# SeoYeonnLee/Video-Chapter-Generation

Measured on AMD Instinct MI355X. Metric: clip-windows/sec (16f×224²+128tok) train-step at 1/2/4/8 MI355X; % HBM roofline, higher is better.
Workload: dtype bf16; 1 GPU; TwoStream train step: TSM-ResNet-50 + BERT-base + ChapterHead(mlp), B=64 windows/GPU of 16x224^2 frames + 128 tokens, fused clip+AdamW; global_batch=64, seq_len=128, frames=16, resolution=224, text_fill=n_valid ~ U[L/2, L], parallelism=dp1

## Files before the change

### video-chapter-generation_amd/csrc/igemm_wide.hip

```cpp
#include "fastload.h"

namespace vcg {

namespace {

__device__ __forceinline__ int w_xcd_slot(int b, int n) {
  const int q = n >> 3, r = n & 7, x = b & 7;
  return (x < r ? x * (q + 1) : r * (q + 1) + (x - r) * q) + (b >> 3);
}

}

enum { WE_STORE = 0, WE_GELU = 1, WE_GELU_BWD = 2, WE_RES = 3, WE_RES32 = 4 };

namespace {

__device__ const float4 g_wide_zero4 = {0.f, 0.f, 0.f, 0.f};

template <int MT, int NT, int WE>
__device__ __forceinline__ void wide_epilogue(f32x4 (&acc)[MT][NT], const GemmParams& p, int m0, int n0) {
  bf16_t* C = reinterpret_cast<bf16_t*>(p.C);
  const bf16_t* R = reinterpret_cast<const bf16_t*>(p.residual);
  float rv[MT][NT][4];
  if constexpr (WE == WE_GELU_BWD || WE == WE_RES || WE == WE_RES32) {
#pragma unroll
    for (int j = 0; j < NT; ++j)
#pragma unroll
      for (int i = 0; i < MT; ++i) {
        const int m = min(m0 + i * 16, p.M - 1), n = min(n0 + j * 16, p.N - 4);
        if constexpr (WE == WE_RES32)
          load4<float>(reinterpret_cast<const float*>(p.residual) + (long long)m * p.ldr + n, rv[i][j]);
        else
          load4<bf16_t>(R + (long long)m * p.ldr + n, rv[i][j]);
      }
  }
#pragma unroll
  for (int j = 0; j < NT; ++j) {
    const int n = n0 + j * 16;
    const float4* bp = p.bias ? reinterpret_cast<const float4*>(p.bias + min(n, p.N - 4)) : &g_wide_zero4;
    const float4 b4 = *bp;
    const float bv[4] = {b4.x, b4.y, b4.z, b4.w};
#pragma unroll
    for (int i = 0; i < MT; ++i) {
      const int m = m0 + i * 16;
      float v[4];
#pragma unroll
      for (int r = 0; r < 4; ++r) {
        float t = acc[i][j][r] + bv[r];
        if constexpr (WE == WE_GELU) {
          v[r] = p.fast_act ? gelu_erf_fast(t) : gelu_erf(t);
          acc[i][j][r] = t;
        } else if constexpr (WE == WE_GELU_BWD) {
          t = bf2f(f2bf(t));
          v[r] = t * (p.fast_act ? gelu_erf_grad_fast(rv[i][j][r]) : gelu_erf_grad(rv[i][j][r]));
        } else if constexpr (WE == WE_RES || WE == WE_RES32) {
          v[r] = t + rv[i][j][r];
        } else {
          v[r] = t;
        }
      }
      if (m < p.M && n < p.N) {
        if constexpr (WE == WE_RES32)
          store4<float>(reinterpret_cast<float*>(p.C) + (long long)m * p.ldc + n, v);
        else
          store4<bf16_t>(C + (long long)m * p.ldc + n, v);
        if constexpr (WE == WE_GELU) {
          if (p.aux) {
            const float a4[4] = {acc[i][j][0], acc[i][j][1], acc[i][j][2], acc[i][j][3]};
            store4<bf16_t>(reinterpret_cast<bf16_t*>(p.aux) + (long long)m * p.ldc + n, a4);
          }
        }
      }
    }
  }
}

}

#ifdef VCG_WIDE_STAMPS
__device__ unsigned long long g_wide_stamps[2 * 16 * 2 * 4];
#define W_STAMP(s, ph, k)                                                                                      \
  do {                                                                                                         \
    if (blockIdx.x == 0 && (tid == 0 || tid == 256) && (s) >= 8 && (s) < 24)                                  \
      g_wide_stamps[((((tid >> 8) * 16 + (s) - 8) * 2 + (ph)) * 4) + (k)] = __builtin_amdgcn_s_memtime();      \
  } while (0)
#else
#define W_STAMP(s, ph, k) do {} while (0)
#endif
#ifndef VCG_WIDE_ABL
#define VCG_WIDE_ABL 0
#endif

template <int P>
__device__ __forceinline__ void wide_wait(int ahead) {
  if (ahead >= 2) __builtin_amdgcn_s_waitcnt(waitcnt_vm(2 * P));
  else if (ahead == 1) __builtin_amdgcn_s_waitcnt(waitcnt_vm(P));
  else __builtin_amdgcn_s_waitcnt(waitcnt_vm(0));
}

template <int BM, int BN, int NW = 8>
struct WideLoader {
  static constexpr int PA = BM / (8 * NW), PB = BN / (8 * NW), P = PA + PB, AE = BM * FBK;
  __amdgpu_buffer_rsrc_t ra, rb;
  uint32_t oa, ob;
  int off[P];
  int kc[P];
  __device__ __forceinline__ void init(const GemmParams& p) {
    oa = (uint32_t)min(p.a.bytes, (long long)0xFFFFFF00LL);
    ob = (uint32_t)min(p.b.bytes, (long long)0xFFFFFF00LL);
    ra = __builtin_amdgcn_make_buffer_rsrc(const_cast<void*>(p.a.ptr), 0, oa, 0x00020000);
    rb = __builtin_amdgcn_make_buffer_rsrc(const_cast<void*>(p.b.ptr), 0, ob, 0x00020000);
  }
  __device__ __forceinline__ void tile(const GemmParams& p, int m0, int n0, int wave, int lane) {
#pragma unroll
    for (int q = 0; q < P; ++q) {
      const bool isa = q < PA;
      const int r = (wave * (isa ? PA : PB) + (isa ? q : q - PA)) * 8 + (lane >> 3);
      kc[q] = 8 * fswz(r, lane & 7);
      const int gr = (isa ? m0 : n0) + r;
      off[q] = gr < (isa ? p.M : p.N) ? (int)((long long)gr * (isa ? p.a.ld : p.b.ld)) + kc[q] : -1;
    }
  }
  template <int Q>
  __device__ __forceinline__ void piece(int k0, int K, bf16_t* stage, int wave) const {
    constexpr bool isa = Q < PA;
    const uint32_t bad = isa ? oa : ob;
    const uint32_t voff = (off[Q] >= 0 && k0 + kc[Q] < K) ? (uint32_t)(off[Q] + k0) * 2u : bad;
    bf16_t* slice = stage + (isa ? 0 : AE) + (wave * (isa ? PA : PB) + (isa ? Q : Q - PA)) * 512;
    __builtin_amdgcn_raw_ptr_buffer_load_lds(isa ? ra : rb, (lds_void_t*)slice, 16, voff, 0, 0, 0);
  }
  template <int Q = 0>
  __device__ __forceinline__ void all(int k0, int K, bf16_t* stage, int wave) const {
    if constexpr (Q < P) {
      piece<Q>(k0, K, stage, wave);
      all<Q + 1>(k0, K, stage, wave);
    }
  }
};

template <int BM, int BN, int WE, int ST = 3>
__global__ __launch_bounds__(512) void gemm_wide_kernel(GemmParams p) {
  constexpr int MT = BM / 32, NT = BN / 64;
  constexpr int AE = BM * FBK, BE = BN * FBK, SE = AE + BE;
  constexpr int PIECES = BM / 64 + BN / 64;
  constexpr int PF = ST - 1;
  static_assert(ST * SE * 2 <= 160 * 1024, "LDS");
  __shared__ __attribute__((aligned(1024))) bf16_t smem[ST * SE];
  const int tid = threadIdx.x, lane = tid & 63;
  const int wave = __builtin_amdgcn_readfirstlane(tid >> 6);
  const int grp = wave >> 2, wc = wave & 3;
  const int ntn = (p.N + BN - 1) / BN, ntm = (p.M + BM - 1) / BM, ntiles = ntn * ntm;
  const int G = gridDim.x;
  const int slot = w_xcd_slot(blockIdx.x, G);
  const int mine = slot < ntiles ? (ntiles - 1 - slot) / G + 1 : 0;
  const int nk = (p.K + FBK - 1) / FBK;
  const int steps = mine * nk;
  if (steps == 0) return;

  WideLoader<BM, BN> ld;
  ld.init(p);
  int ikt = 0, itile = 0;
  bf16_t* istage = smem;
  auto next_tile = [&]() {
    if (ikt == 0) {
      const int L = slot + itile * G, mt = L / ntn, nt = L - mt * ntn;
      ld.tile(p, mt * BM, nt * BN, wave, lane);
    }
  };
  auto advance = [&]() {
    if (++ikt == nk) {
      ikt = 0;
      ++itile;
    }
  };

  f32x4 acc[MT][NT];
#pragma unroll
  for (int i = 0; i < MT; ++i)
#pragma unroll
    for (int j = 0; j < NT; ++j) acc[i][j] = f32x4{0.f, 0.f, 0.f, 0.f};

#pragma unroll
  for (int t = 0; t < PF; ++t)
    if (t < steps) {
      next_tile();
      ld.all(ikt * FBK, p.K, smem + t * SE, wave);
      advance();
    }
  wide_wait<PIECES>(min(PF, steps) - 1);
  __builtin_amdgcn_s_barrier();
  if (grp == 1) __builtin_amdgcn_s_barrier();

  int cur = 0, kt = 0, tile = 0;
  s16x8 af[MT][2], bq[NT][2];
  for (int s = 0; s < steps; ++s) {
    const bf16_t* Ac = smem + cur * SE;
    const bf16_t* Bc = Ac + AE;
    const bool pre = s + PF < steps;
    if (pre) {
      next_tile();
      istage = smem + (cur == 0 ? ST - 1 : cur - 1) * SE;
    }
    const int ik0 = ikt * FBK;
    W_STAMP(s, 0, 0);
    if (VCG_WIDE_ABL != 3 || s == 0) {
#pragma unroll
      for (int s2 = 0; s2 < 2; ++s2) {
#pragma unroll
        for (int j = 0; j < NT; ++j) bq[j][s2] = fast_frag(Bc, wc * (BN / 4) + j * 16, lane, s2);
#pragma unroll
        for (int i = 0; i < MT; ++i) af[i][s2] = fast_frag(Ac, grp * (BM / 2) + i * 16, lane, s2);
      }
    }
    if (pre && VCG_WIDE_ABL != 1) ld.all(ik0, p.K, istage, wave);
    W_STAMP(s, 0, 1);
    __builtin_amdgcn_s_waitcnt(0xC07F);
    W_STAMP(s, 0, 2);
    if (grp == 1 && s + 1 < steps && VCG_WIDE_ABL != 1)
      wide_wait<PIECES>(min(s + PF, steps - 1) - (s + 1));
    W_STAMP(s, 0, 3);
    __builtin_amdgcn_s_barrier();
    W_STAMP(s, 1, 0);
    __builtin_amdgcn_sched_barrier(0);
    __builtin_amdgcn_s_setprio(1);
    if (VCG_WIDE_ABL != 2) {
#pragma unroll
      for (int s2 = 0; s2 < 2; ++s2)
#pragma unroll
        for (int i = 0; i < MT; ++i)
#pragma unroll
          for (int j = 0; j < NT; ++j)
            acc[i][j] = __builtin_amdgcn_mfma_f32_16x16x32_bf16(bq[j][s2], af[i][s2], acc[i][j], 0, 0, 0);
    }
    __builtin_amdgcn_s_setprio(0);
    if (pre) advance();
    W_STAMP(s, 1, 1);
    if (grp == 0 && s + 1 < steps && VCG_WIDE_ABL != 1) wide_wait<PIECES>(min(s + PF, steps - 1) - (s + 1));
    W_STAMP(s, 1, 2);
    __builtin_amdgcn_sched_barrier(0);
    if (++kt == nk) {
      const int L = slot + tile * G, mt = L / ntn, nt = L - mt * ntn;
      wide_epilogue<MT, NT, WE>(acc, p, mt * BM + grp * (BM / 2) + (lane & 15), nt * BN + wc * (BN / 4) + 4 * (lane >> 4));
#pragma unroll
      for (int i = 0; i < MT; ++i)
#pragma unroll
        for (int j = 0; j < NT; ++j) acc[i][j] = f32x4{0.f, 0.f, 0.f, 0.f};
      kt = 0;
      ++tile;
    }
    W_STAMP(s, 1, 3);
    __builtin_amdgcn_s_barrier();
    cur = cur == ST - 1 ? 0 : cur + 1;
  }
  if (grp == 0) __builtin_amdgcn_s_barrier();
}

namespace {

int wide_cus() {
  static int n = 0;
  if (n == 0) {
    int dev = 0, c = 0;
    if (hipGetDevice(&dev) == hipSuccess && hipDeviceGetAttribute(&c, hipDeviceAttributeMultiprocessorCount, dev) ==
                                                hipSuccess && c > 0)
      n = c;
    else
      n = 256;
  }
  return n;
}

int wide_bn_for(const GemmParams& p) {
  if (const char* e = getenv("VCG_WIDE_BN")) {
    const int v = atoi(e);
    if (v == 128 || v == 192 || v == 256) return v;
  }
  if (p.N >= 3072 && p.N % 256 == 0) return 256;
  return p.N % 192 == 0 ? 192 : 128;
}

template <int BN, int WE>
void launch_wide(const GemmParams& p, hipStream_t s) {
  constexpr int BM = 128;
  const long long tiles = (long long)((p.M + BM - 1) / BM) * ((p.N + BN - 1) / BN);
  const int grid = (int)(tiles < wide_cus() ? tiles : wide_cus());
  hipLaunchKernelGGL((gemm_wide_kernel<BM, BN, WE>), dim3(grid), dim3(512), 0, s, p);
}

template <int BN>
void launch_wide_we(const GemmParams& p, int we, hipStream_t s) {
  switch (we) {
    case WE_GELU: launch_wide<BN, WE_GELU>(p, s); break;
    case WE_GELU_BWD: launch_wide<BN, WE_GELU_BWD>(p, s); break;
    case WE_RES: launch_wide<BN, WE_RES>(p, s); break;
    case WE_RES32: launch_wide<BN, WE_RES32>(p, s); break;
    default: launch_wide<BN, WE_STORE>(p, s); break;
  }
}

}

int wide_gemm_class(const GemmParams& p) {
  if (p.alpha != 1.f || p.batch_inner > 0 || p.M <= 0 || p.N <= 0 || p.K <= 0) return -1;
  if (p.N % 8 != 0 || p.K % 8 != 0 || (p.ldc & 7) != 0 || (p.a.ld & 7) != 0 || (p.b.ld & 7) != 0) return -1;
  if ((((uintptr_t)p.C | (uintptr_t)p.a.ptr | (uintptr_t)p.b.ptr) & 15) != 0) return -1;
  if (p.a.bytes >= 0xFFFFFF00LL || p.b.bytes >= 0xFFFFFF00LL) return -1;
  if (p.bias && ((uintptr_t)p.bias & 15) != 0) return -1;
  if (p.aux && (p.act != ACT_GELU || ((uintptr_t)p.aux & 15) != 0)) return -1;
  if (p.residual) {
    if (p.residual == p.C || (p.ldr & 3) != 0 || ((uintptr_t)p.residual & 7) != 0) return -1;
    if (p.act == ACT_GELU_BWD) return WE_GELU_BWD;
    return p.act == ACT_NONE && !p.res_round ? WE_RES : -1;
  }
  if (p.act == ACT_GELU) return WE_GELU;
  return p.act == ACT_NONE ? WE_STORE : -1;
}

int wide_gemm_class_f32(const GemmParams& p) {
  if (!p.residual || p.aux || p.act != ACT_NONE || p.res_round || p.alpha != 1.f || p.batch_inner > 0) return -1;
  if (p.N % 8 != 0 || p.K % 8 != 0 || (p.ldc & 3) != 0 || (p.ldr & 3) != 0 || (p.a.ld & 7) != 0 || (p.b.ld & 7) != 0)
    return -1;
  if ((((uintptr_t)p.C | (uintptr_t)p.residual | (uintptr_t)p.a.ptr | (uintptr_t)p.b.ptr) & 15) != 0) return -1;
  if (p.a.bytes >= 0xFFFFFF00LL || p.b.bytes >= 0xFFFFFF00LL) return -1;
  if (p.bias && ((uintptr_t)p.bias & 15) != 0) return -1;
  return WE_RES32;
}

int run_gemm_wide(GemmParams& p, int we, hipStream_t s) {
  const int tk = timing_begin(s);
  switch (wide_bn_for(p)) {
    case 128: launch_wide_we<128>(p, we, s); break;
    case 256: launch_wide_we<256>(p, we, s); break;
    default: launch_wide_we<192>(p, we, s); break;
  }
  const double es = we == WE_RES32 ? 4.0 : 2.0;
  double bytes = 2.0 * ((double)p.M * p.K + (double)p.N * p.K) + es * p.M * (double)p.N;
  if (p.residual) bytes += es * p.M * (double)p.N;
  if (p.aux) bytes += 2.0 * p.M * (double)p.N;
  timing_end(tk, s, TIMING_WIDE_GEMM, 2.0 * p.M * p.N * (double)p.K, bytes);
  if (census_on()) { char t_[96]; snprintf(t_, sizeof(t_), "gemm_wide 128x%d we%d", wide_bn_for(p), we); census_add(t_, p.M, p.N, p.K); }
  VCG_LAUNCH_CHECK();
  return VCG_OK;
}

}

VCG_API int vcg_wide_stamps(unsigned long long* out, int n) {
#ifdef VCG_WIDE_STAMPS
  n = n < 256 ? n : 256;
  return hipMemcpyFromSymbol(out, HIP_SYMBOL(vcg::g_wide_stamps), (size_t)n * 8, 0, hipMemcpyDeviceToHost) == hipSuccess
             ? 0 : 2;
#else
  (void)out;
  (void)n;
  return 1;
#endif
}
```

Measured before the change: 913.0 clip-windows/sec.

## Restructure wide GEMM main loop to overlap fragment loads with MFMA halves

Reworks the persistent wide GEMM loop so each k-step splits into two MFMA halves. The second-half LDS fragments are read while the first half computes, and the next stage's first-half fragments are read after the barrier. Global prefetch is now issued after compute into the just-consumed stage, one barrier per step replaces the staggered group barriers, and bias/residual loads for the epilogue are issued early on the last k-step with vmcnt accounting. This is meant to hide LDS and epilogue load latency, but it relies on hand-counted waitcnts that are fixed to 3 stages.

```diff
diff --git a/video-chapter-generation_amd/csrc/igemm_wide.hip b/video-chapter-generation_amd/csrc/igemm_wide.hip
--- a/video-chapter-generation_amd/csrc/igemm_wide.hip
+++ b/video-chapter-generation_amd/csrc/igemm_wide.hip
@@ -1,3 +1,5 @@
+#include <type_traits>
+
 #include "fastload.h"
 
 namespace vcg {
@@ -15,30 +17,74 @@
 
 namespace {
 
-__device__ const float4 g_wide_zero4 = {0.f, 0.f, 0.f, 0.f};
-
-template <int MT, int NT, int WE>
-__device__ __forceinline__ void wide_epilogue(f32x4 (&acc)[MT][NT], const GemmParams& p, int m0, int n0) {
+
+template <int WE> struct WideRes { using T = uint2; };
+template <> struct WideRes<WE_RES32> { using T = float4; };
+constexpr bool wide_has_res(int we) { return we == WE_GELU_BWD || we == WE_RES || we == WE_RES32; }
+
+template <int MT, int NT, int WE>
+struct WideEpiOps {
+  float4 bias[NT];
+  typename WideRes<WE>::T res[MT][NT];
+};
+template <int MT, int NT, int WE>
+constexpr bool wide_res_early() {
+  return wide_has_res(WE) && MT * NT * (int)sizeof(typename WideRes<WE>::T) / 4 <= 48;
+}
+template <int MT, int NT, int WE>
+constexpr int wide_epi_loads() { return NT + (wide_res_early<MT, NT, WE>() ? MT * NT : 0); }
+
+template <int MT, int NT, int WE>
+__device__ __forceinline__ void wide_res_load(WideEpiOps<MT, NT, WE>& e, const GemmParams& p, int m0, int n0) {
+  using T = typename WideRes<WE>::T;
+  const char* R = reinterpret_cast<const char*>(p.residual);
+#pragma unroll
+  for (int j = 0; j < NT; ++j)
+#pragma unroll
+    for (int i = 0; i < MT; ++i) {
+      const int m = min(m0 + i * 16, p.M - 1), n = min(n0 + j * 16, p.N - 4);
+      e.res[i][j] = *reinterpret_cast<const T*>(R + ((long long)m * p.ldr + n) * (long long)(sizeof(T) / 4));
+    }
+}
+
+template <int MT, int NT, int WE>
+__device__ __forceinline__ void wide_epi_load(WideEpiOps<MT, NT, WE>& e, const GemmParams& p, int m0, int n0) {
+#pragma unroll
+  for (int j = 0; j < NT; ++j) {
+    const float* bp = p.bias ? p.bias + min(n0 + j * 16, p.N - 4) : reinterpret_cast<const float*>(p.a.ptr);
+    e.bias[j] = *reinterpret_cast<const float4*>(bp);
+  }
+  if constexpr (wide_res_early<MT, NT, WE>()) wide_res_load<MT, NT, WE>(e, p, m0, n0);
+}
+
+__device__ __forceinline__ void wide_res_f32(const uint2& q, float (&v)[4]) {
+  v[0] = __uint_as_float(q.x << 16); v[1] = __uint_as_float(q.x & 0xffff0000u);
+  v[2] = __uint_as_float(q.y << 16); v[3] = __uint_as_float(q.y & 0xffff0000u);
+}
+__device__ __forceinline__ void wide_res_f32(const float4& q, float (&v)[4]) {
+  v[0] = q.x; v[1] = q.y; v[2] = q.z; v[3] = q.w;
+}
+
+template <int MT, int NT, int WE>
+__device__ __forceinline__ void wide_epilogue(f32x4 (&acc)[MT][NT], WideEpiOps<MT, NT, WE>& e,
+                                              const GemmParams& p, int m0, int n0) {
   bf16_t* C = reinterpret_cast<bf16_t*>(p.C);
-  const bf16_t* R = reinterpret_cast<const bf16_t*>(p.residual);
   float rv[MT][NT][4];
-  if constexpr (WE == WE_GELU_BWD || WE == WE_RES || WE == WE_RES32) {
+  if constexpr (wide_has_res(WE) && !wide_res_early<MT, NT, WE>()) {
+    wide_res_load<MT, NT, WE>(e, p, m0, n0);
+    __builtin_amdgcn_s_waitcnt(waitcnt_vm(0));
+  }
+  if constexpr (wide_has_res(WE)) {
 #pragma unroll
     for (int j = 0; j < NT; ++j)
 #pragma unroll
-      for (int i = 0; i < MT; ++i) {
-        const int m = min(m0 + i * 16, p.M - 1), n = min(n0 + j * 16, p.N - 4);
-        if constexpr (WE == WE_RES32)
-          load4<float>(reinterpret_cast<const float*>(p.residual) + (long long)m * p.ldr + n, rv[i][j]);
-        else
-          load4<bf16_t>(R + (long long)m * p.ldr + n, rv[i][j]);
-      }
-  }
+      for (int i = 0; i < MT; ++i) wide_res_f32(e.res[i][j], rv[i][j]);
+  }
+  const bool has_bias = p.bias != nullptr;
 #pragma unroll
   for (int j = 0; j < NT; ++j) {
     const int n = n0 + j * 16;
-    const float4* bp = p.bias ? reinterpret_cast<const float4*>(p.bias + min(n, p.N - 4)) : &g_wide_zero4;
-    const float4 b4 = *bp;
+    const float4 b4 = has_bias ? e.bias[j] : float4{0.f, 0.f, 0.f, 0.f};
     const float bv[4] = {b4.x, b4.y, b4.z, b4.w};
 #pragma unroll
     for (int i = 0; i < MT; ++i) {
@@ -91,11 +137,16 @@
 #define VCG_WIDE_ABL 0
 #endif
 
-template <int P>
+template <int P, int X = 0>
 __device__ __forceinline__ void wide_wait(int ahead) {
-  if (ahead >= 2) __builtin_amdgcn_s_waitcnt(waitcnt_vm(2 * P));
-  else if (ahead == 1) __builtin_amdgcn_s_waitcnt(waitcnt_vm(P));
-  else __builtin_amdgcn_s_waitcnt(waitcnt_vm(0));
+  static_assert(2 * P + X <= 63, "vmcnt");
+  if (ahead >= 2) __builtin_amdgcn_s_waitcnt(waitcnt_vm(2 * P + X));
+  else if (ahead == 1) __builtin_amdgcn_s_waitcnt(waitcnt_vm(P + X));
+  else __builtin_amdgcn_s_waitcnt(waitcnt_vm(X));
+}
+
+__device__ __forceinline__ constexpr int waitcnt_lgkm(int n) {
+  return 0xF | (0x7 << 4) | ((n & 0xF) << 8) | (0x3 << 14);
 }
 
 template <int BM, int BN, int NW = 8>
@@ -143,7 +194,8 @@
   constexpr int MT = BM / 32, NT = BN / 64;
   constexpr int AE = BM * FBK, BE = BN * FBK, SE = AE + BE;
   constexpr int PIECES = BM / 64 + BN / 64;
-  constexpr int PF = ST - 1;
+  constexpr int NE = wide_epi_loads<MT, NT, WE>();
+  static_assert(ST == 3, "the waits below count for 3 stages");
   static_assert(ST * SE * 2 <= 160 * 1024, "LDS");
   __shared__ __attribute__((aligned(1024))) bf16_t smem[ST * SE];
   const int tid = threadIdx.x, lane = tid & 63;
@@ -160,14 +212,12 @@
   WideLoader<BM, BN> ld;
   ld.init(p);
   int ikt = 0, itile = 0;
-  bf16_t* istage = smem;
-  auto next_tile = [&]() {
+  auto issue = [&](bf16_t* stage) {
     if (ikt == 0) {
       const int L = slot + itile * G, mt = L / ntn, nt = L - mt * ntn;
       ld.tile(p, mt * BM, nt * BN, wave, lane);
     }
-  };
-  auto advance = [&]() {
+    ld.all(ikt * FBK, p.K, stage, wave);
     if (++ikt == nk) {
       ikt = 0;
       ++itile;
@@ -181,78 +231,107 @@
     for (int j = 0; j < NT; ++j) acc[i][j] = f32x4{0.f, 0.f, 0.f, 0.f};
 
 #pragma unroll
-  for (int t = 0; t < PF; ++t)
-    if (t < steps) {
-      next_tile();
-      ld.all(ikt * FBK, p.K, smem + t * SE, wave);
-      advance();
-    }
-  wide_wait<PIECES>(min(PF, steps) - 1);
+  for (int t = 0; t < ST; ++t)
+    if (t < steps) issue(smem + t * SE);
+  wide_wait<PIECES>(min(ST, steps) - 1);
   __builtin_amdgcn_s_barrier();
-  if (grp == 1) __builtin_amdgcn_s_barrier();
-
-  int cur = 0, kt = 0, tile = 0;
+  __builtin_amdgcn_sched_barrier(0);
+
+  const int wm = grp * (BM / 2), wn = wc * (BN / 4);
   s16x8 af[MT][2], bq[NT][2];
-  for (int s = 0; s < steps; ++s) {
-    const bf16_t* Ac = smem + cur * SE;
-    const bf16_t* Bc = Ac + AE;
-    const bool pre = s + PF < steps;
-    if (pre) {
-      next_tile();
-      istage = smem + (cur == 0 ? ST - 1 : cur - 1) * SE;
-    }
-    const int ik0 = ikt * FBK;
+#pragma unroll
+  for (int j = 0; j < NT; ++j) bq[j][0] = fast_frag(smem + AE, wn + j * 16, lane, 0);
+#pragma unroll
+  for (int i = 0; i < MT; ++i) af[i][0] = fast_frag(smem, wm + i * 16, lane, 0);
+
+  int cur = 0, tile = 0, s = 0;
+  auto kstep = [&](auto last_c) {
+    constexpr bool last = decltype(last_c)::value;
+    WideEpiOps<MT, NT, WE> eo;
+    bf16_t* stage = smem + cur * SE;
+    const int nxt = cur == ST - 1 ? 0 : cur + 1;
+    const bool more = s + 1 < steps, pre = s + ST < steps;
+    const int L = slot + tile * G, mt = L / ntn, nt = L - mt * ntn;
+    const int em = mt * BM + wm + (lane & 15), en = nt * BN + wn + 4 * (lane >> 4);
+    if constexpr (last) wide_epi_load<MT, NT, WE>(eo, p, em, en);
+    __builtin_amdgcn_sched_barrier(0);
     W_STAMP(s, 0, 0);
     if (VCG_WIDE_ABL != 3 || s == 0) {
 #pragma unroll
-      for (int s2 = 0; s2 < 2; ++s2) {
-#pragma unroll
-        for (int j = 0; j < NT; ++j) bq[j][s2] = fast_frag(Bc, wc * (BN / 4) + j * 16, lane, s2);
-#pragma unroll
-        for (int i = 0; i < MT; ++i) af[i][s2] = fast_frag(Ac, grp * (BM / 2) + i * 16, lane, s2);
-      }
-    }
-    if (pre && VCG_WIDE_ABL != 1) ld.all(ik0, p.K, istage, wave);
+      for (int j = 0; j < NT; ++j) bq[j][1] = fast_frag(stage + AE, wn + j * 16, lane, 1);
+#pragma unroll
+      for (int i = 0; i < MT; ++i) af[i][1] = fast_frag(stage, wm + i * 16, lane, 1);
+    }
+    __builtin_amdgcn_sched_barrier(0);
+    __builtin_amdgcn_s_waitcnt(waitcnt_lgkm(MT + NT));
+    __builtin_amdgcn_sched_barrier(0);
     W_STAMP(s, 0, 1);
-    __builtin_amdgcn_s_waitcnt(0xC07F);
+    __builtin_amdgcn_s_setprio(1);
+    if (VCG_WIDE_ABL != 2) {
+#pragma unroll
+      for (int i = 0; i < MT; ++i)
+#pragma unroll
+        for (int j = 0; j < NT; ++j)
+          acc[i][j] = __builtin_amdgcn_mfma_f32_16x16x32_bf16(bq[j][0], af[i][0], acc[i][j], 0, 0, 0);
+    }
+    __builtin_amdgcn_s_setprio(0);
+    __builtin_amdgcn_sched_barrier(0);
     W_STAMP(s, 0, 2);
-    if (grp == 1 && s + 1 < steps && VCG_WIDE_ABL != 1)
-      wide_wait<PIECES>(min(s + PF, steps - 1) - (s + 1));
+    __builtin_amdgcn_s_waitcnt(waitcnt_lgkm(0));
+    if (more && VCG_WIDE_ABL != 1) {
+      const int ahead = min(s + 2, steps - 1) - (s + 1);
+      if constexpr (last) wide_wait<PIECES, NE>(ahead);
+      else wide_wait<PIECES>(ahead);
+    }
     W_STAMP(s, 0, 3);
     __builtin_amdgcn_s_barrier();
+    __builtin_amdgcn_sched_barrier(0);
     W_STAMP(s, 1, 0);
-    __builtin_amdgcn_sched_barrier(0);
+    if (more && VCG_WIDE_ABL != 3) {
+      const bf16_t* An = smem + nxt * SE;
+#pragma unroll
+      for (int j = 0; j < NT; ++j) bq[j][0] = fast_frag(An + AE, wn + j * 16, lane, 0);
+#pragma unroll
+      for (int i = 0; i < MT; ++i) af[i][0] = fast_frag(An, wm + i * 16, lane, 0);
+    }
+    __builtin_amdgcn_sched_barrier(0);
+    W_STAMP(s, 1, 1);
     __builtin_amdgcn_s_setprio(1);
     if (VCG_WIDE_ABL != 2) {
 #pragma unroll
-      for (int s2 = 0; s2 < 2; ++s2)
-#pragma unroll
-        for (int i = 0; i < MT; ++i)
-#pragma unroll
-          for (int j = 0; j < NT; ++j)
-            acc[i][j] = __builtin_amdgcn_mfma_f32_16x16x32_bf16(bq[j][s2], af[i][s2], acc[i][j], 0, 0, 0);
+      for (int i = 0; i < MT; ++i)
+#pragma unroll
+        for (int j = 0; j < NT; ++j)
+          acc[i][j] = __builtin_amdgcn_mfma_f32_16x16x32_bf16(bq[j][1], af[i][1], acc[i][j], 0, 0, 0);
     }
     __builtin_amdgcn_s_setprio(0);
-    if (pre) advance();
-    W_STAMP(s, 1, 1);
-    if (grp == 0 && s + 1 < steps && VCG_WIDE_ABL != 1) wide_wait<PIECES>(min(s + PF, steps - 1) - (s + 1));
+    __builtin_amdgcn_sched_barrier(0);
+    if constexpr (!last) {
+      if (pre && VCG_WIDE_ABL != 1) issue(stage);
+    }
+    __builtin_amdgcn_sched_barrier(0);
     W_STAMP(s, 1, 2);
-    __builtin_amdgcn_sched_barrier(0);
-    if (++kt == nk) {
-      const int L = slot + tile * G, mt = L / ntn, nt = L - mt * ntn;
-      wide_epilogue<MT, NT, WE>(acc, p, mt * BM + grp * (BM / 2) + (lane & 15), nt * BN + wc * (BN / 4) + 4 * (lane >> 4));
+    if constexpr (last) {
+      __builtin_amdgcn_s_waitcnt(waitcnt_vm(0));
+      wide_epilogue<MT, NT, WE>(acc, eo, p, em, en);
 #pragma unroll
       for (int i = 0; i < MT; ++i)
 #pragma unroll
         for (int j = 0; j < NT; ++j) acc[i][j] = f32x4{0.f, 0.f, 0.f, 0.f};
-      kt = 0;
       ++tile;
+      __builtin_amdgcn_sched_barrier(0);
+      if (pre && VCG_WIDE_ABL != 1) issue(stage);
+      __builtin_amdgcn_s_waitcnt(waitcnt_lgkm(0));
     }
     W_STAMP(s, 1, 3);
-    __builtin_amdgcn_s_barrier();
-    cur = cur == ST - 1 ? 0 : cur + 1;
-  }
-  if (grp == 0) __builtin_amdgcn_s_barrier();
+    cur = nxt;
+    ++s;
+  };
+  __builtin_amdgcn_s_waitcnt(waitcnt_lgkm(0));
+  for (int t = 0; t < mine; ++t) {
+    for (int k = 1; k < nk; ++k) kstep(std::false_type{});
+    kstep(std::true_type{});
+  }
 }
 
 namespace {
```

Result: no change. 917.5 clip-windows/sec (median of 6 runs) (+0.5%).
